# Unrepentant-Atheist/AC-3-ACM-Codec

Measured on AMD Instinct MI355X. Metric: AC-3 5.1@48kHz frames/sec/GPU (decode+encode); achieved HBM GB/s vs peak, higher is better.
Workload: dtype f32+i32

## Files before the change

ac-3-acm-codec_amd/capi.py:

```python
import ctypes
import os
import re

_HERE = os.path.dirname(os.path.abspath(__file__))
LIB_PATH = os.environ.get("AC3MI_LIB") or os.path.join(_HERE, "libac3mi.so")
HEADER_DIR = os.path.join(os.path.dirname(_HERE), "include")

c_void_p, c_int, c_float, c_size_t, c_char_p = (ctypes.c_void_p, ctypes.c_int, ctypes.c_float,
                                                ctypes.c_size_t, ctypes.c_char_p)


class AC3MIError(RuntimeError):
    pass


class XformDescC(ctypes.Structure):
    _fields_ = [("acmod", c_int), ("lfeon", c_int), ("output", c_int), ("bias", c_float)]


class DecodeDescC(ctypes.Structure):
    _fields_ = [("flags", c_int), ("level", c_float), ("bias", c_float), ("dynrng", c_int),
                ("acmod", c_int), ("lfeon", c_int), ("frame_bytes", c_int)]


# ... 179 lines not shown
    lib.ac3mi_syncinfo.argtypes = [c_void_p, ctypes.POINTER(c_int), ctypes.POINTER(c_int), ctypes.POINTER(c_int)]
    lib.ac3mi_decode_planes.argtypes = [ctypes.POINTER(DecodeDescC), ctypes.POINTER(c_int), ctypes.POINTER(c_int)]
    lib.ac3mi_decode_batch.argtypes = [c_void_p, ctypes.POINTER(DecodeDescC), c_void_p, c_int, c_int, c_int,
                                       c_void_p, c_void_p, c_void_p, c_void_p, ctypes.POINTER(DecodeTapsC)]
    lib.ac3mi_decode_s16_batch.argtypes = [c_void_p, ctypes.POINTER(DecodeDescC), c_void_p, c_int, c_int, c_int,
                                           c_void_p, c_void_p, c_void_p, c_void_p]
    lib.ac3mi_encode_frame_bytes.argtypes = [ctypes.POINTER(EncodeDescC)]
    lib.ac3mi_encode_tables.argtypes = [c_void_p] * 5
    lib.ac3mi_encode_batch.argtypes = [c_void_p, ctypes.POINTER(EncodeDescC), c_void_p, c_void_p, c_void_p, c_void_p,
                                       c_void_p, c_int, c_int, c_int, ctypes.POINTER(EncodeTapsC)]
    lib.ac3mi_set_decode_mode.argtypes = [c_void_p, ctypes.c_int]
    if hasattr(lib, "ac3mi_set_fixed_shape"):
        lib.ac3mi_set_fixed_shape.argtypes = [c_void_p, ctypes.c_int]
    if hasattr(lib, "ac3mi_fill_workspaces"):
        lib.ac3mi_fill_workspaces.argtypes = [c_void_p, ctypes.c_int]
    lib.ac3mi_set_decode_crc.argtypes = [c_void_p, ctypes.c_int]
    lib.ac3mi_crc_check_batch.argtypes = [c_void_p, c_void_p, c_int, c_int, c_size_t, c_void_p]
    lib.ac3mi_set_mix_state.argtypes = [c_void_p, c_void_p, c_void_p]
    lib.ac3mi_probe_valu_rate.argtypes = [c_void_p, ctypes.POINTER(ctypes.c_double)]
    lib.ac3mi_probe_salu_rate.argtypes = [c_void_p, ctypes.POINTER(ctypes.c_double)]
    lib.ac3mi_probe_mixed_rate.argtypes = [c_void_p, ctypes.c_int, ctypes.POINTER(ctypes.c_double), ctypes.POINTER(ctypes.c_double)]
    lib.ac3mi_probe_copy_rate.argtypes = [c_void_p, ctypes.c_size_t, ctypes.POINTER(ctypes.c_double)]
    lib.ac3mi_set_tile_frames.argtypes = [c_void_p, ctypes.c_longlong]
    lib.ac3mi_transcode_batch.argtypes = [c_void_p, ctypes.POINTER(DecodeDescC), ctypes.POINTER(EncodeDescC), c_void_p, ctypes.c_int,
                                          ctypes.c_int, ctypes.c_int, c_void_p, c_void_p, c_void_p, c_void_p, c_void_p, c_void_p,
                                          ctypes.c_int, c_void_p]
    _lib = lib
    return lib
```

ac-3-acm-codec_amd/csrc/ac3mi_internal.h:

```cpp
#pragma once
#include <hip/hip_runtime.h>
#include <stdint.h>
#include <array>
#include <string>
#include "../../include/ac3mi.h"
#include "launch_rule.h"

namespace ac3mi {

struct DecTables {
    int8_t la_neg[256];
    uint16_t hth[3][50];
    int8_t width[64];
    uint8_t band_end[30];
    uint8_t band_of_bin[256];
    float qlev[48];
    float qtab[760];
    uint32_t desc[128];
};

struct EncTables {
    int16_t win[256];
    int16_t cos[64], sin[64];
    int16_t xcos[128], xsin[128];
// ... 216 lines not shown
    uint8_t *frames;
    int frame_stride, n_streams, frames_per_stream;
    uint8_t chmap[8];
    int32_t *ws_mdct;
    bool mdct_full_rows = false;
    uint8_t *ws_expo;
    int8_t *ws_shift;
    uint8_t *ws_eexp;
    int16_t *ws_emask;
    uint8_t *ws_strat;
    int32_t *ws_ebits;
    int32_t *ws_snr;
    uint32_t *ws_memo;
    uint8_t *tap_eexp, *tap_bap, *tap_strat;
    int32_t *tap_snr;
    const int32_t *slot;
    int pack_mode = 0;
    const uint32_t *search_hint = nullptr;
    int search_hint_stride = 0;
    uint8_t *ws_bsw = nullptr;
    uint8_t *ws_remat = nullptr;
    int cpl_begf = -1;
    CplWs ws_cpl = {};
    int chbwcod = 50;
    bool bw = false;
    uint32_t bsi = BSI_DEFAULT;
    const uint32_t *bsi_words = nullptr;
    int drc_profile = 0;
    int32_t *drc_state = nullptr;
    int16_t *ws_drc_gain = nullptr;
// ... 62 lines not shown
    ac3mi::DevBuf ws_crc;
    ac3mi::DevBuf ws_bsi;
    ac3mi::DevBuf ws_dyn;
    template <class Ctx> static auto workspaces(Ctx *c)
    {
        return std::array{&c->ws_coef, &c->ws_blksw, &c->ws_draws, &c->ws_split, &c->ws_enc, &c->ws_tc,
                          &c->ws_bsw, &c->ws_remat, &c->ws_cpl, &c->ws_cplr, &c->ws_drc, &c->ws_crc, &c->ws_bsi, &c->ws_dyn};
    }
    const int32_t *slots = nullptr;
    float *mix_pending = nullptr;
    int32_t *mix_flags = nullptr;
    long long tile_frames = 131072;
    int decode_mode = 0;
    int decode_crc = 0;
    int fixed_shape = 1;
    double *loud_tab = nullptr;
    std::string err;
};
```

ac-3-acm-codec_amd/csrc/capi.hip:

```cpp
#include "ac3mi_internal.h"
#include "a52_levels.h"
#include "spec_tables.h"
#include "sync_rule.h"
#include <math.h>
#include <stdio.h>
#include <string.h>
#include <vector>

namespace ac3mi {

static std::string g_err;



static double bessel_i0(double x)
{
    double b = 1;
    for (int i = 100; i > 0; i--) b = b * x / (i * i) + 1;
    return b;
}

void build_host_tables(float *window, float2 *tw_long, float2 *tw_short)
{
    const double pi = 3.14159265358979323846;
// ... 647 lines not shown

int ac3mi_set_decode_mode(ac3mi_ctx *ctx, int mode)
{
    if (!ctx || mode < 0 || mode > 6 || mode == 2) return AC3MI_ERR_ARG;
    ctx->decode_mode = mode;
    return AC3MI_OK;
}

int ac3mi_set_fixed_shape(ac3mi_ctx *ctx, int on)
{
    if (!ctx || on < 0 || on > 1) return AC3MI_ERR_ARG;
    ctx->fixed_shape = on;
    return AC3MI_OK;
}

int ac3mi_set_decode_crc(ac3mi_ctx *ctx, int mode)
{
    if (!ctx || mode < 0 || mode > 2) return AC3MI_ERR_ARG;
    ctx->decode_crc = mode;
    return AC3MI_OK;
}

int ac3mi_set_encode_mode(ac3mi_ctx *ctx, int mode)
{
    if (!ctx || mode < 0 || mode > 2) return AC3MI_ERR_ARG;
    ctx->encode_mode = mode;
    return AC3MI_OK;
}

int ac3mi_set_encode_block_switch(ac3mi_ctx *ctx, int mode)
// ... 346 lines not shown
    E.ws_ebits = ctx->ws_enc.at<int32_t>(W.off_ebits);
    E.ws_snr = ctx->ws_enc.at<int32_t>(W.off_snr);
    E.ws_memo = ctx->ws_enc.at<uint32_t>(W.off_memo);
    if (taps && taps->d_mdct) { E.ws_mdct = taps->d_mdct; E.mdct_full_rows = true; }
    if (taps && taps->d_exponent) E.ws_expo = taps->d_exponent;
    if (taps && taps->d_exp_samples) E.ws_shift = taps->d_exp_samples;
    if (taps && taps->d_encoded_exp) E.ws_eexp = taps->d_encoded_exp;
    E.tap_eexp = taps ? taps->d_encoded_exp : nullptr;
    E.tap_bap = taps ? taps->d_bap : nullptr;
    E.tap_strat = taps ? taps->d_exp_strategy : nullptr;
    E.tap_snr = taps ? taps->d_snroffst : nullptr;
    E.chbwcod = call_chbwcod(ctx, desc, E.cfg.nfbw);
    E.bw = t.bw_mode != 0;
    E.exp_strategy = t.exp_strategy;
    E.pack_mode = ctx->encode_mode;
    E.fixed_shape = ctx->fixed_shape != 0;
    E.slot = ctx->slots;
    return AC3MI_OK;
}

size_t ac3mi_transcode_workspace_plan(size_t frames, int frames_per_stream, int n_in, int nfchans, int n_out)
{
    const bool mantx = dec_mantx(0, frames_per_stream, n_in == n_out, true);
    return (mantx ? 0 : coef_bytes(frames, n_in)) + (zs_off(frames, nfchans) + frames) + split_bytes(frames) +
           s16_ws_bytes(frames, n_out) + enc_ws_layout(frames * 6 * (size_t)n_out).need;
}

int ac3mi_xform_planes(const ac3mi_xform_desc *desc, int *n_in, int *n_out)
{
    MixPlan plan;
    if (!desc) return AC3MI_ERR_ARG;
// ... 640 lines not shown
```

ac-3-acm-codec_amd/csrc/encode.hip:

```cpp
#include "ac3mi_internal.h"
#include "wave_ops.h"
#include "spec_tables.h"
#include "enc_mant.h"
#include "enc_syntax.h"

#include <type_traits>

namespace ac3mi {

#define WAVE_SYNC()                                          \
    do {                                                     \
        __builtin_amdgcn_fence(__ATOMIC_RELEASE, "wavefront"); \
        __builtin_amdgcn_wave_barrier();                     \
        __builtin_amdgcn_fence(__ATOMIC_ACQUIRE, "wavefront"); \
    } while (0)

__device__ __forceinline__ int ilog2u(unsigned v) { return v ? 31 - __builtin_clz(v) : 0; }

__device__ __forceinline__ int wave_sum(int v) { return (int)wave_sum_u32((uint32_t)v); }


struct PackParams {
    const int32_t *mdct;
    const uint8_t *eexp;
    const int16_t *emask;
    const uint8_t *strat;
    const int32_t *ebits;
    const int8_t *shift;
    int32_t *csnr_state;
    const int32_t *slot;
    int32_t *snr;
    uint32_t *memo;
    uint8_t *frames;
    const EncTables *tab;
    uint8_t *tap_eexp;
    uint8_t *tap_bap;
    uint8_t *tap_strat;
    int32_t *tap_snr;
    int n_streams, frames_per_stream, frame_stride;
    int nch, nfbw, lfe, acmod, fscod, halfrate, bsid, frmsizecod, frame_words;
    int nbc;
    int chbwcod;
    uint16_t crc_inv_t[16];
    uint16_t pw1_t[6][16], pw2_t[6][16];
    int c1, c2;
    int frw;
    int marker;
    const uint32_t *hint;
    int hint_stride;
    const uint8_t *bsw;
    const uint8_t *remat;
    CplWs cpl;
    int cpl_begf;
// ... 21 lines not shown
__device__ __forceinline__ uint32_t pack_dynrng(const PackParams &P, size_t fidx, int b, int p)
{
    if constexpr (DW) if (P.dyn) return dyn_sends(P.dyn + fidx * 12, b, p) ? 0x100u | P.dyn[fidx * 12 + 2 * b + p] : 0u;
    if constexpr (MD) if (P.drc && drc_sends(P.drc + fidx * 6, b)) return 0x100u | P.drc[fidx * 6 + b];
    return 0u;
}

struct MaskTabs {
    uint8_t latab[256];
    uint16_t hth[50];
    uint8_t band_of_bin[256];
    uint8_t band_start[52];
};

template <bool CPL>
struct alignas(16) SearchLDS {
    int16_t mask[CPL ? 42 : 36][50];
    uint32_t bitlut[64];
    uint8_t strat[6][6];
    uint8_t band_of_bin[256];
    uint32_t rowdesc[CPL ? 42 : 36];
    uint2 terms[2][50];
};

__device__ __forceinline__ void put_bits(uint32_t *fr, int frw, uint32_t pos, int n, uint32_t v)
{
    if (n <= 0) return;
    const uint32_t w = pos >> 5;
    if (w + 1 >= (uint32_t)frw) return;
    const uint64_t x = (uint64_t)v << (64 - n - (pos & 31));
    const uint32_t hi = (uint32_t)(x >> 32), lo = (uint32_t)x;
    if (hi) atomicOr(&fr[w], hi);
// ... 1315 lines not shown
#define PK_DECL() do { } while (0)
#define PK_T0() do { } while (0)
#define PK_LAP(id) do { } while (0)
#define PK_COUNT(id) do { } while (0)
#define PK_END() do { } while (0)
#endif

#ifndef ENC_NC
#define ENC_NC 3
#endif

#ifndef ENC_SEARCH_LB
#define ENC_SEARCH_LB 4
#endif
template <int PART, bool CPL = false, bool BW = false, bool DRC = false, bool FX = false, bool DW = false>
__global__ __launch_bounds__(64, ENC_SEARCH_LB) void enc_search_kernel(const PackParams P)
{
    static_assert(PART == 1 || PART == 3, "the packers are enc_packf_kernel / enc_packb_kernel");
    static_assert(!DW || DRC, "the array words are costed where the profiles' are");
    static_assert(!FX || (PART == 1 && !CPL && !BW && !DRC), "the fixed 5.1 shape is the plain per-stream search's");
    __shared__ SearchLDS<CPL> L;
    const int lane = threadIdx.x;
    constexpr bool PER_FRAME = PART == 3;
    const int s = PER_FRAME ? (int)(blockIdx.x / (unsigned)P.frames_per_stream) : (int)blockIdx.x;
    const int f_first = PER_FRAME ? (int)(blockIdx.x - (unsigned)s * (unsigned)P.frames_per_stream) : 0;
    const int f_end = PER_FRAME ? f_first + 1 : FX ? 1 : P.frames_per_stream;
    if (s >= P.n_streams) return;

    for (int i = lane; i < 256; i += 64) L.band_of_bin[i] = P.tab->band_of_bin[i];
    {
        const int bp = P.tab->baptab[lane];
        L.bitlut[lane] = (uint32_t)plain_bits(bp) | ((bp == 1) << 9) | ((bp == 2) << 14) | ((bp == 4) << 19);
    }

    const int nch = FX ? 6 : P.nch, nfbw = FX ? 5 : P.nfbw, nbc = FX ? 223 : P.nbc;
    const int acmod = FX ? 7 : P.acmod;
    const bool lfe = FX ? true : P.lfe != 0;
    const int fs = P.frame_words;

    const int sslot = P.slot ? P.slot[s] : s;
    const int cpl_cs = 37 + 12 * P.cpl_begf;
    const int cpl_ce = BW ? 73 + 12 * P.cpl_endf : 217, cpl_nb = BW ? 3 + P.cpl_endf - P.cpl_begf : 15 - P.cpl_begf;
    const int state_in = P.csnr_state[sslot];
    int csnr_prev = state_in & 0xff, fsnr_prev = (state_in >> 8) & 15;
    PK_DECL();

    for (int f = f_first; f < f_end; f++) {
        const size_t fidx = FX ? (size_t)s : (size_t)s * P.frames_per_stream + f;
        PK_T0();
        PK_COUNT(5);
        const uint8_t *ex = P.eexp + fidx * 6 * nch * 256;
        int frame_bits = 0;
        uint64_t run_starts = 0, row_set = 0;
        int ncplrows = 0;
        const bool cplf = CPL && (__builtin_amdgcn_readfirstlane((int)P.cpl.word[fidx]) & 1);
        const uint8_t *cex = cplf ? P.cpl.eexp + fidx * 6 * 256 : ex;
        bool loaded = false;
        auto load_frame = [&]() {
            loaded = true;
            {
                const uint32_t *gm = reinterpret_cast<const uint32_t *>(P.emask + fidx * 6 * nch * 50);
                uint32_t mv[15];
#pragma unroll
                for (int j = 0; j < 15; j++) {
                    const int i = lane + 64 * j;
                    mv[j] = i < 6 * nch * 25 ? gm[i] : 0;
                }
#pragma unroll
                for (int j = 0; j < 15; j++) {
                    const int i = lane + 64 * j;
                    if (i < 6 * nch * 25) reinterpret_cast<uint32_t *>(&L.mask[0][0])[i] = mv[j];
                }
            }
            if (lane < 6 * nch) { const int b = lane / nch, ch = lane - b * nch; L.strat[b][ch] = P.strat[fidx * 6 * nch + lane]; }
            frame_bits = wave_sum(lane < nch ? P.ebits[fidx * nch + lane] : 0);
// ... 30 lines not shown
                    }
                    for (int p = 0; p < np; p++) frame_bits += (compr_word(P, fidx, p) & 0x100u) ? 8 : 0;
                }
                if (!FX && P.remat)
                    for (int b = 1; b < 6; b++) frame_bits += (P.remat[fidx * 6 + b] & 0x10) ? 4 : 0;
                if (CPL && cplf) {
                    frame_bits += syn_priced_cpl(acmod, nfbw, cpl_nb);
                    frame_bits += __builtin_amdgcn_readfirstlane(P.cpl.ebits[fidx]) - 6 * __builtin_popcountll(row_set & fbw_rows);
                    if (P.remat) {
                        const int nrem = syn_cpl_nrem(P.cpl_begf);
                        for (int b = 1; b < 6; b++) frame_bits -= (P.remat[fidx * 6 + b] & 0x10) ? 4 - nrem : 0;
                    }
                }
            }
            if constexpr (CPL) if (cplf) {
                const uint32_t *gm = reinterpret_cast<const uint32_t *>(P.cpl.emask + fidx * 6 * 50);
                for (int i = lane; i < 150; i += 64) reinterpret_cast<uint32_t *>(&L.mask[36][0])[i] = gm[i];
                const int st = lane < 6 ? (int)P.cpl.strat[fidx * 8 + lane] : 0;
                const uint32_t cst = (uint32_t)__ballot(lane < 6 && st != 0) | 0x40u;
                const int n0 = __builtin_popcountll(row_set);
                if (lane < 6 && st != 0) {
                    const int b1 = __builtin_ctz(cst >> (lane + 1)) + lane + 1;
                    const uint32_t cover = ((1u << b1) - 1u) & ~((1u << lane) - 1u);
                    L.rowdesc[n0 + __builtin_popcount(cst & ((1u << lane) - 1u))] = (uint32_t)(lane * 256) | (1u << 15) | (cover << 16) | ((uint32_t)(36 + lane) << 24);
                }
                ncplrows = __builtin_popcount(cst & 0x3fu);
                WAVE_SYNC();
            }
        };
        if (PART != 1 || (!FX && P.tap_strat)) load_frame();

        const uint32_t bandoff = *reinterpret_cast<const uint32_t *>(&L.band_of_bin[4 * lane]);
        SnrSearch ss{csnr_prev, 0, 0, false};
        uint64_t known_c = 0, fits_c = 0;
        uint32_t known_f = 0, fits_f = 0;
        int f_cc = -1;
        if (PART == 1 && !FX && P.memo) {
            const uint32_t *m = P.memo + fidx * 8;
            auto word = [&](int i) { return (uint32_t)__builtin_amdgcn_readfirstlane((int)m[i]); };
            known_c = (uint64_t)word(0) | ((uint64_t)word(1) << 32);
            fits_c = (uint64_t)word(2) | ((uint64_t)word(3) << 32);
            known_f = word(4);
            fits_f = word(5);
            f_cc = (int)word(6);
        }
// ... 3 lines not shown
        int gl = -1, spare_l = 0, gh = -1, spare_h = 0;
        int probe_sweeps = 0;
        auto lookup = [&](int cc, int ff, bool &fits) {
            const int g = 16 * cc + ff;
            if (g <= fit_hi) { fits = true; return true; }
            if (g >= fail_lo) { fits = false; return true; }
            if (((uint32_t)__builtin_amdgcn_readlane((int)costed_map, g >> 5) >> (g & 31)) & 1u) {
                fits = ((uint32_t)__builtin_amdgcn_readlane((int)fits_map, g >> 5) >> (g & 31)) & 1u;
                return true;
            }
            if (ff == 0) { fits = (fits_c >> cc) & 1; return (bool)((known_c >> cc) & 1); }
            fits = (fits_f >> ff) & 1;
            return cc == f_cc && ((known_f >> ff) & 1);
        };
        auto cost_and_record = [&](const int (&cg)[ENC_NC], int n_cand, bool probing) {
            if (!loaded) load_frame();
            int so[ENC_NC];
#pragma unroll
            for (int k = 0; k < ENC_NC; k++) so[k] = ((k < n_cand ? cg[k] : cg[0]) - 240) << 2;
            PK_COUNT(4);
            const int budget = 16 * fs - frame_bits;
            uint32_t acc[6][ENC_NC];
#pragma unroll
            for (int B = 0; B < 6; B++)
#pragma unroll
                for (int c = 0; c < ENC_NC; c++) acc[B][c] = 0;
            {
                const int nrows = __builtin_popcountll(row_set) + (CPL ? ncplrows : 0);
                auto desc_of = [&](int i) { return (uint32_t)__builtin_amdgcn_readfirstlane((int)L.rowdesc[i < nrows ? i : nrows - 1]); };
                auto fetch = [&](uint32_t d) {
// ... 110 lines not shown
                    costed_map |= bit;
                    fits_map |= ok ? bit : 0u;
                }
                {
                    const bool up = ok && g > gl, dn = !ok && (gh < 0 || g < gh);
                    gl = up ? g : gl; spare_l = up ? spare : spare_l;
                    gh = dn ? g : gh; spare_h = dn ? spare : spare_h;
                }
                if (cand_fi == 0) { known_c |= 1ull << cand_ci; fits_c |= (uint64_t)ok << cand_ci; }
                else if (!probing || cand_ci == f_cc) {
                    if (cand_ci != f_cc) { f_cc = cand_ci; known_f = fits_f = 0; }
                    known_f |= 1u << cand_fi;
                    fits_f |= (uint32_t)ok << cand_fi;
                }
            }
        };
        bool first_sweep = true;
        const bool cold_hint = csnr_prev == 40 && fsnr_prev == 0;
        for (;;) {
            int cc, ff;
            bool more;
            while ((more = ss.next(cc, ff))) {
                bool fits;
                if (!lookup(cc, ff, fits)) break;
                if (ss.phase == 0 && !fits) went_down = true;
                if (ss.phase == 1 && fits) went_up = true;
                ss.consume(fits);
            }
            if (!more) break;
            int cg[ENC_NC], n_cand = 0;
#pragma unroll
            for (int k = 0; k < ENC_NC; k++) cg[k] = -1;
            auto add = [&](int g) {
// ... 749 lines not shown
    PackParams P;
    P.mdct = E.ws_mdct;
    P.eexp = E.ws_eexp;
    P.emask = E.ws_emask;
    P.strat = E.ws_strat;
    P.ebits = E.ws_ebits;
    P.shift = E.ws_shift;
    P.csnr_state = E.csnr;
    P.slot = E.slot;
    P.frames = E.frames;
    P.tab = tab.enc;
    P.tap_eexp = E.tap_eexp;
    P.tap_bap = E.tap_bap;
    P.tap_strat = E.tap_strat;
    P.tap_snr = E.tap_snr;
    P.n_streams = E.n_streams;
    P.frames_per_stream = E.frames_per_stream;
    P.frame_stride = E.frame_stride;
    P.nch = c.nch;
    P.nfbw = c.nfbw;
    P.lfe = c.lfe;
    P.acmod = c.acmod;
    P.fscod = c.fscod;
    P.halfrate = c.halfrate;
    P.bsid = c.bsid;
    P.frmsizecod = c.frmsizecod;
    P.frame_words = c.frame_words;
    P.nbc = R.nbc;
    P.chbwcod = E.chbwcod;
    const int fs = c.frame_words, fs58 = (fs >> 1) + (fs >> 3);
// ... 93 lines not shown
```

ac-3-acm-codec_amd/csrc/wave_ops.h:

```cpp
#pragma once
#include <hip/hip_runtime.h>
#include <stdint.h>

namespace ac3mi {

__device__ __forceinline__ uint32_t wave_incl_scan_u32(uint32_t v)
{
    v += (uint32_t)__builtin_amdgcn_update_dpp(0, (int)v, 0x111, 0xf, 0xf, true);
    v += (uint32_t)__builtin_amdgcn_update_dpp(0, (int)v, 0x112, 0xf, 0xf, true);
    v += (uint32_t)__builtin_amdgcn_update_dpp(0, (int)v, 0x114, 0xf, 0xf, true);
    v += (uint32_t)__builtin_amdgcn_update_dpp(0, (int)v, 0x118, 0xf, 0xf, true);
    v += (uint32_t)__builtin_amdgcn_update_dpp(0, (int)v, 0x142, 0xa, 0xf, false);
    v += (uint32_t)__builtin_amdgcn_update_dpp(0, (int)v, 0x143, 0xc, 0xf, false);
    return v;
}

__device__ __forceinline__ uint32_t wave_last(uint32_t v) { return (uint32_t)__builtin_amdgcn_readlane((int)v, 63); }

__device__ __forceinline__ uint32_t wave_sum_u32(uint32_t v) { return wave_last(wave_incl_scan_u32(v)); }

__device__ __forceinline__ uint32_t wave_or_u32(uint32_t v)
{
    v |= (uint32_t)__builtin_amdgcn_update_dpp(0, (int)v, 0x111, 0xf, 0xf, true);
    v |= (uint32_t)__builtin_amdgcn_update_dpp(0, (int)v, 0x112, 0xf, 0xf, true);
    v |= (uint32_t)__builtin_amdgcn_update_dpp(0, (int)v, 0x114, 0xf, 0xf, true);
    v |= (uint32_t)__builtin_amdgcn_update_dpp(0, (int)v, 0x118, 0xf, 0xf, true);
    v |= (uint32_t)__builtin_amdgcn_update_dpp(0, (int)v, 0x142, 0xa, 0xf, false);
    v |= (uint32_t)__builtin_amdgcn_update_dpp(0, (int)v, 0x143, 0xc, 0xf, false);
// ... 65 lines not shown
```

ac-3-acm-codec_amd/engine.py:

```python
import ctypes
from dataclasses import dataclass

from . import capi


@dataclass
class XformDesc:
    acmod: int = 7
    lfeon: int = 1
    output: int = 7 | 16
    bias: float = 0.0

    def c(self):
        return capi.XformDescC(self.acmod, self.lfeon, self.output, self.bias)


@dataclass
class DecodeDesc:
    flags: int = 7 | 16
    level: float = 1.0
    bias: float = 0.0
    dynrng: int = 1
    acmod: int = 7
    lfeon: int = 1
# ... 300 lines not shown
        self.lib.ac3mi_workspace_bytes.restype = ctypes.c_size_t
        return int(self.lib.ac3mi_workspace_bytes(ctypes.c_void_p(self.ctx)))

    def fill_workspaces(self, byte):
        self._check(self.lib.ac3mi_fill_workspaces(ctypes.c_void_p(self.ctx), int(byte)))

    def set_tile_frames(self, frames):
        self._check(self.lib.ac3mi_set_tile_frames(ctypes.c_void_p(self.ctx), int(frames)))

    def set_decode_mode(self, mode):
        self._check(self.lib.ac3mi_set_decode_mode(ctypes.c_void_p(self.ctx), int(mode)))

    def set_fixed_shape(self, on):
        self._check(self.lib.ac3mi_set_fixed_shape(ctypes.c_void_p(self.ctx), int(on)))

    def set_decode_crc(self, mode):
        self._check(self.lib.ac3mi_set_decode_crc(ctypes.c_void_p(self.ctx), int(mode)))

    def crc_check_batch(self, frames, frame_bytes=None, out=None, wait_torch=True):
        import torch
        assert frames.dtype == torch.uint8 and frames.is_contiguous() and frames.is_cuda and frames.dim() >= 2
        stride = frames.shape[-1]
        n = frames.numel() // stride if stride else 0
        if out is None:
            out = torch.zeros(tuple(frames.shape[:-1]), dtype=torch.uint8, device=frames.device)
        assert out.dtype == torch.uint8 and out.is_contiguous() and out.numel() == n
        self._drain_torch(wait_torch)
        self._check(self.lib.ac3mi_crc_check_batch(ctypes.c_void_p(self.ctx), ctypes.c_void_p(frames.data_ptr()), int(stride),
                                                   int(stride if frame_bytes is None else frame_bytes), ctypes.c_size_t(n),
                                                   ctypes.c_void_p(out.data_ptr())))
# ... 279 lines not shown
```

include/ac3mi.h:

```cpp
#ifndef AC3MI_H
#define AC3MI_H

#include <stddef.h>
#include <stdint.h>

#ifdef __cplusplus
extern "C" {
#endif

#define AC3MI_CHANNEL 0
#define AC3MI_MONO 1
#define AC3MI_STEREO 2
#define AC3MI_3F 3
#define AC3MI_2F1R 4
#define AC3MI_3F1R 5
#define AC3MI_2F2R 6
#define AC3MI_3F2R 7
#define AC3MI_CHANNEL1 8
#define AC3MI_CHANNEL2 9
#define AC3MI_DOLBY 10
#define AC3MI_CHANNEL_MASK 15
#define AC3MI_LFE 16
#define AC3MI_ADJUST_LEVEL 32

// ... 33 lines not shown
    int output;
    float bias;
} ac3mi_xform_desc;

int ac3mi_set_state_slots(ac3mi_ctx *ctx, const int32_t *d_slots);

int ac3mi_set_mix_state(ac3mi_ctx *ctx, float *d_pending, int32_t *d_flags);

#define AC3MI_STATUS_REUSE0 0x200u
int ac3mi_set_decode_mode(ac3mi_ctx *ctx, int mode);

int ac3mi_set_fixed_shape(ac3mi_ctx *ctx, int on);

int ac3mi_fill_workspaces(ac3mi_ctx *ctx, int byte);

#define AC3MI_STATUS_CRC1 0x400u
#define AC3MI_STATUS_CRC2 0x800u
int ac3mi_set_decode_crc(ac3mi_ctx *ctx, int mode);

int ac3mi_crc_check_batch(ac3mi_ctx *ctx, const uint8_t *d_frames, int frame_stride, int frame_bytes, size_t n_frames,
                          uint8_t *d_verdict);

#define AC3MI_BSI_NOT_READ 0x80u
#define AC3MI_BSI_OVERRUN 0x40u
#define AC3MI_BSI_COMPRE 0x001u
#define AC3MI_BSI_LANGCODE 0x002u
#define AC3MI_BSI_AUDPRODIE 0x004u
#define AC3MI_BSI_COMPR2E 0x008u
#define AC3MI_BSI_LANGCOD2E 0x010u
#define AC3MI_BSI_AUDPRODI2E 0x020u
// ... 207 lines not shown
```

Measured before the change: 9.294 million.

## Cost sixteen SNR offsets per sweep with histogram window search in encoder

Replaces the per-candidate bit costing in the per-stream encoder SNR search (PART 1) with a windowed sweep. Each pass costs 16 consecutive SNR offsets at once using wave scans and LDS histograms of the bit-count steps, and a predictive rule (linear interpolation, hints) picks the next window. The mask rows are no longer staged in LDS; masks are read straight from global memory. Launch bounds for the fixed 5.1 shape go up to 7 waves per EU, and a debug curve tap plus a Python simulator are added. This aims to cut the number of search iterations per frame, at the cost of more per-sweep work and register pressure.

```diff
diff --git a/ac-3-acm-codec_amd/capi.py b/ac-3-acm-codec_amd/capi.py
--- a/ac-3-acm-codec_amd/capi.py
+++ b/ac-3-acm-codec_amd/capi.py
@@ -217,6 +217,8 @@
         lib.ac3mi_set_fixed_shape.argtypes = [c_void_p, ctypes.c_int]
     if hasattr(lib, "ac3mi_fill_workspaces"):
         lib.ac3mi_fill_workspaces.argtypes = [c_void_p, ctypes.c_int]
+    if hasattr(lib, "ac3mi_debug_search_curve"):
+        lib.ac3mi_debug_search_curve.argtypes = [c_void_p, c_void_p]
     lib.ac3mi_set_decode_crc.argtypes = [c_void_p, ctypes.c_int]
     lib.ac3mi_crc_check_batch.argtypes = [c_void_p, c_void_p, c_int, c_int, c_size_t, c_void_p]
     lib.ac3mi_set_mix_state.argtypes = [c_void_p, c_void_p, c_void_p]
diff --git a/ac-3-acm-codec_amd/csrc/ac3mi_internal.h b/ac-3-acm-codec_amd/csrc/ac3mi_internal.h
--- a/ac-3-acm-codec_amd/csrc/ac3mi_internal.h
+++ b/ac-3-acm-codec_amd/csrc/ac3mi_internal.h
@@ -254,6 +254,7 @@
     uint32_t *ws_memo;
     uint8_t *tap_eexp, *tap_bap, *tap_strat;
     int32_t *tap_snr;
+    int32_t *tap_curve = nullptr;
     const int32_t *slot;
     int pack_mode = 0;
     const uint32_t *search_hint = nullptr;
@@ -346,6 +347,7 @@
     int decode_mode = 0;
     int decode_crc = 0;
     int fixed_shape = 1;
+    int32_t *debug_search_curve = nullptr;
     double *loud_tab = nullptr;
     std::string err;
 };
diff --git a/ac-3-acm-codec_amd/csrc/capi.hip b/ac-3-acm-codec_amd/csrc/capi.hip
--- a/ac-3-acm-codec_amd/csrc/capi.hip
+++ b/ac-3-acm-codec_amd/csrc/capi.hip
@@ -685,6 +685,13 @@
     return AC3MI_OK;
 }
 
+int ac3mi_debug_search_curve(ac3mi_ctx *ctx, int32_t *d_curve)
+{
+    if (!ctx) return AC3MI_ERR_ARG;
+    ctx->debug_search_curve = d_curve;
+    return AC3MI_OK;
+}
+
 int ac3mi_set_decode_crc(ac3mi_ctx *ctx, int mode)
 {
     if (!ctx || mode < 0 || mode > 2) return AC3MI_ERR_ARG;
@@ -1061,7 +1068,8 @@
     E.bw = t.bw_mode != 0;
     E.exp_strategy = t.exp_strategy;
     E.pack_mode = ctx->encode_mode;
-    E.fixed_shape = ctx->fixed_shape != 0;
+    E.tap_curve = ctx->debug_search_curve;
+    E.fixed_shape = ctx->fixed_shape != 0 && !ctx->debug_search_curve;
     E.slot = ctx->slots;
     return AC3MI_OK;
 }
diff --git a/ac-3-acm-codec_amd/csrc/encode.hip b/ac-3-acm-codec_amd/csrc/encode.hip
--- a/ac-3-acm-codec_amd/csrc/encode.hip
+++ b/ac-3-acm-codec_amd/csrc/encode.hip
@@ -3,6 +3,7 @@
 #include "spec_tables.h"
 #include "enc_mant.h"
 #include "enc_syntax.h"
+#include "snr_window.h"
 
 #include <type_traits>
 
@@ -37,6 +38,7 @@
     uint8_t *tap_bap;
     uint8_t *tap_strat;
     int32_t *tap_snr;
+    int32_t *tap_curve;
     int n_streams, frames_per_stream, frame_stride;
     int nch, nfbw, lfe, acmod, fscod, halfrate, bsid, frmsizecod, frame_words;
     int nbc;
@@ -88,8 +90,15 @@
 };
 
 template <bool CPL>
-struct alignas(16) SearchLDS {
+struct SearchMaskRows {
     int16_t mask[CPL ? 42 : 36][50];
+};
+struct SearchWindowBufs {
+    alignas(16) uint32_t scan[4 + 256];
+    alignas(16) uint32_t hist[4][6][15][2];
+};
+template <bool CPL, bool WIN>
+struct alignas(16) SearchLDS : std::conditional_t<WIN, SearchWindowBufs, SearchMaskRows<CPL>> {
     uint32_t bitlut[64];
     uint8_t strat[6][6];
     uint8_t band_of_bin[256];
@@ -1435,12 +1444,13 @@
 #define ENC_SEARCH_LB 4
 #endif
 template <int PART, bool CPL = false, bool BW = false, bool DRC = false, bool FX = false, bool DW = false>
-__global__ __launch_bounds__(64, ENC_SEARCH_LB) void enc_search_kernel(const PackParams P)
+__global__ __launch_bounds__(64, FX ? 7 : ENC_SEARCH_LB) void enc_search_kernel(const PackParams P)
 {
     static_assert(PART == 1 || PART == 3, "the packers are enc_packf_kernel / enc_packb_kernel");
     static_assert(!DW || DRC, "the array words are costed where the profiles' are");
     static_assert(!FX || (PART == 1 && !CPL && !BW && !DRC), "the fixed 5.1 shape is the plain per-stream search's");
-    __shared__ SearchLDS<CPL> L;
+    constexpr bool WIN = PART == 1;
+    __shared__ SearchLDS<CPL, WIN> L;
     const int lane = threadIdx.x;
     constexpr bool PER_FRAME = PART == 3;
     const int s = PER_FRAME ? (int)(blockIdx.x / (unsigned)P.frames_per_stream) : (int)blockIdx.x;
@@ -1452,6 +1462,13 @@
     {
         const int bp = P.tab->baptab[lane];
         L.bitlut[lane] = (uint32_t)plain_bits(bp) | ((bp == 1) << 9) | ((bp == 2) << 14) | ((bp == 4) << 19);
+    }
+    int band_lo = 0, band_hi = 0;
+    if constexpr (WIN) {
+        const int b = lane < 50 ? lane : 49;
+        band_lo = 3 + P.tab->band_start[b];
+        band_hi = 3 + (b < 49 ? P.tab->band_start[b + 1] : 256);
+        if (lane == 0) L.scan[3] = 0;
     }
 
     const int nch = FX ? 6 : P.nch, nfbw = FX ? 5 : P.nfbw, nbc = FX ? 223 : P.nbc;
@@ -1479,7 +1496,7 @@
         bool loaded = false;
         auto load_frame = [&]() {
             loaded = true;
-            {
+            if constexpr (!WIN) {
                 const uint32_t *gm = reinterpret_cast<const uint32_t *>(P.emask + fidx * 6 * nch * 50);
                 uint32_t mv[15];
 #pragma unroll
@@ -1540,8 +1557,10 @@
                 }
             }
             if constexpr (CPL) if (cplf) {
-                const uint32_t *gm = reinterpret_cast<const uint32_t *>(P.cpl.emask + fidx * 6 * 50);
-                for (int i = lane; i < 150; i += 64) reinterpret_cast<uint32_t *>(&L.mask[36][0])[i] = gm[i];
+                if constexpr (!WIN) {
+                    const uint32_t *gm = reinterpret_cast<const uint32_t *>(P.cpl.emask + fidx * 6 * 50);
+                    for (int i = lane; i < 150; i += 64) reinterpret_cast<uint32_t *>(&L.mask[36][0])[i] = gm[i];
+                }
                 const int st = lane < 6 ? (int)P.cpl.strat[fidx * 8 + lane] : 0;
                 const uint32_t cst = (uint32_t)__ballot(lane < 6 && st != 0) | 0x40u;
                 const int n0 = __builtin_popcountll(row_set);
@@ -1554,7 +1573,7 @@
                 WAVE_SYNC();
             }
         };
-        if (PART != 1 || (!FX && P.tap_strat)) load_frame();
+        if (PART != 1 || FX || P.tap_strat) load_frame();
 
         const uint32_t bandoff = *reinterpret_cast<const uint32_t *>(&L.band_of_bin[4 * lane]);
         SnrSearch ss{csnr_prev, 0, 0, false};
@@ -1588,6 +1607,7 @@
             return cc == f_cc && ((known_f >> ff) & 1);
         };
         auto cost_and_record = [&](const int (&cg)[ENC_NC], int n_cand, bool probing) {
+          if constexpr (!WIN) {
             if (!loaded) load_frame();
             int so[ENC_NC];
 #pragma unroll
@@ -1728,9 +1748,188 @@
                     fits_f |= (uint32_t)ok << cand_fi;
                 }
             }
+          }
+        };
+        int win_sweeps = 0, win_slope15 = 0, win_cmin = 1 << 20, win_cmax = -1;
+        auto cost_window = [&](int lo) {
+          if constexpr (WIN) {
+            if (!loaded) load_frame();
+            PK_COUNT(4);
+            const int so_lo = win_snroffset(lo);
+            const int budget = 16 * fs - frame_bits;
+            uint32_t acc[6];
+#pragma unroll
+            for (int B = 0; B < 6; B++) acc[B] = 0;
+            static_assert(sizeof L.hist == 180 * sizeof(uint4), "cleared as 180 uint4");
+#pragma unroll
+            for (int i = 0; i < 3; i++)
+                if (lane + 64 * i < 180) reinterpret_cast<uint4 *>(&L.hist[0][0][0][0])[lane + 64 * i] = make_uint4(0, 0, 0, 0);
+            {
+                const int nrows = __builtin_popcountll(row_set) + (CPL ? ncplrows : 0);
+                auto desc_of = [&](int i) { return (uint32_t)__builtin_amdgcn_readfirstlane((int)L.rowdesc[i < nrows ? i : nrows - 1]); };
+                auto fetch = [&](uint32_t d) {
+                    if constexpr (CPL) return *reinterpret_cast<const uint32_t *>(((d & (1u << 15)) ? cex : ex) + (d & 0x3fffu) + 4 * lane);
+                    else return *reinterpret_cast<const uint32_t *>(ex + (d & 0x3fffu) + 4 * lane);
+                };
+                const int bl = lane < 50 ? lane : 49;
+                const int16_t *gmask = P.emask + fidx * 6 * nch * 50 + bl;
+                auto mask_of = [&](uint32_t d) {
+                    if constexpr (CPL) if (d & (1u << 15)) return (int)P.cpl.emask[(fidx * 6 + ((d >> 24) - 36)) * 50 + bl];
+                    return (int)gmask[(d >> 24) * 50u];
+                };
+                uint32_t d0 = desc_of(0), d1 = desc_of(1), d2 = desc_of(2);
+                uint32_t ev = fetch(d0), ev1 = fetch(d1), ev2 = fetch(d2);
+                int t1c = 0, t2c = 0;
+                auto terms = [&](int m, int buf, int &t1, int &t2) {
+                    int k0;
+                    win_steps(m - so_lo, k0, t1, t2);
+                    const int D = win_term(k0);
+                    if (lane < 50) L.terms[buf][lane] = make_uint2((uint32_t)(D & 0xffff) | ((uint32_t)(D + 4) << 16), (uint32_t)((D + 8) & 0xffff));
+                };
+                int mv1 = mask_of(d1);
+                terms(mask_of(d0), 0, t1c, t2c);
+                auto beyond = [&](int n) { const int k = n - 4 * lane; return k >= 4 ? 0u : k <= 0 ? 0xffffffffu : 0xffffffffu << (8 * k); };
+                const uint32_t um_fbw = beyond(nbc), um_lfe = beyond(7);
+                uint32_t boff[4];
+#pragma unroll
+                for (int j = 0; j < 4; j++) boff[j] = ((bandoff >> (8 * j)) & 0xffu) * 8u;
+#pragma unroll 1
+                for (int i = 0; i < nrows; i++) {
+                    const uint32_t d3 = desc_of(i + 3);
+                    const uint32_t ev3 = fetch(d3);
+                    const int mv2 = mask_of(d2);
+                    const char *Tr = reinterpret_cast<const char *>(&L.terms[i & 1][0]);
+                    uint32_t em;
+                    if constexpr (CPL) {
+                        const uint32_t um_cch = beyond(cpl_cs), um_cpl = ~beyond(cpl_cs) | beyond(cpl_ce);
+                        em = ev | ((d0 & (1u << 14)) ? um_lfe : (d0 & (1u << 15)) ? um_cpl : (d0 & (1u << 22)) ? um_cch : um_fbw);
+                    } else {
+                        em = ev | ((d0 & (1u << 14)) ? um_lfe : um_fbw);
+                    }
+                    uint32_t p[3][4];
+#pragma unroll
+                    for (int j = 0; j < 4; j++) {
+                        const uint32_t e16 = __umul24((em >> (8 * j)) & 0xffu, 0x00100010u);
+                        const uint2 t = *reinterpret_cast<const uint2 *>(Tr + boff[j]);
+                        pk2 a01 = __builtin_bit_cast(pk2, t.x) - __builtin_bit_cast(pk2, e16);
+                        pk2 a2 = __builtin_bit_cast(pk2, t.y) - __builtin_bit_cast(pk2, e16);
+                        a01 = __builtin_elementwise_min(__builtin_elementwise_max(a01, (pk2){0, 0}), (pk2){252, 252});
+                        a2 = __builtin_elementwise_min(__builtin_elementwise_max(a2, (pk2){0, 0}), (pk2){252, 252});
+                        const char *lut = reinterpret_cast<const char *>(&L.bitlut[0]);
+                        const uint32_t v0 = *reinterpret_cast<const uint32_t *>(lut + (uint16_t)a01.x);
+                        const uint32_t v1 = *reinterpret_cast<const uint32_t *>(lut + (uint16_t)a01.y);
+                        const uint32_t v2 = *reinterpret_cast<const uint32_t *>(lut + (uint16_t)a2.x);
+                        p[0][j] = j ? p[0][j - 1] + v0 : v0;
+                        p[1][j] = j ? p[1][j - 1] + v1 : v1;
+                        p[2][j] = j ? p[2][j - 1] + v2 : v2;
+                    }
+#pragma unroll
+                    for (int B = 0; B < 6; B++) {
+                        const uint32_t in_run = (d0 >> (16 + B)) & 1u;
+                        asm("v_mad_u32_u24 %0, %1, %2, %0" : "+v"(acc[B]) : "v"(p[0][3]), "s"(in_run));
+                    }
+                    uint32_t W[3];
+#pragma unroll
+                    for (int c = 0; c < 3; c++) {
+                        const uint32_t incl = wave_incl_scan_u32(p[c][3]);
+                        const uint32_t before = incl - p[c][3];
+                        *reinterpret_cast<uint4 *>(&L.scan[4 + 4 * lane]) = make_uint4(before + p[c][0], before + p[c][1], before + p[c][2], incl);
+                        W[c] = L.scan[band_hi] - L.scan[band_lo];
+                    }
+                    {
+                        const uint32_t cover = (d0 >> 16) & 0x3fu;
+                        const int b_in = __builtin_ctz(cover), b_out = b_in + __builtin_popcount(cover);
+                        const uint32_t a0 = win_wide_a(W[0]), a1 = win_wide_a(W[1]), a2 = win_wide_a(W[2]);
+                        const uint32_t b0 = win_wide_b(W[0]), b1 = win_wide_b(W[1]), b2 = win_wide_b(W[2]);
+                        const bool s1 = lane < 50 && t1c < WIN_N && ((a1 ^ a0) | (b1 ^ b0)) != 0, s2 = lane < 50 && t2c < WIN_N && ((a2 ^ a1) | (b2 ^ b1)) != 0;
+                        uint32_t *h1 = &L.hist[lane & 3][b_in][s1 ? t1c - 1 : 0][0], *h2 = &L.hist[lane & 3][b_in][s2 ? t2c - 1 : 0][0];
+                        if (s1) { atomicAdd(h1, a1 - a0); atomicAdd(h1 + 1, b1 - b0); }
+                        if (s2) { atomicAdd(h2, a2 - a1); atomicAdd(h2 + 1, b2 - b1); }
+                        if (b_out < 6) {
+                            const int behind = (b_out - b_in) * 30;
+                            if (s1) { atomicAdd(h1 + behind, a0 - a1); atomicAdd(h1 + behind + 1, b0 - b1); }
+                            if (s2) { atomicAdd(h2 + behind, a1 - a2); atomicAdd(h2 + behind + 1, b1 - b2); }
+                        }
+                    }
+                    if (i + 1 < nrows) terms(mv1, (i + 1) & 1, t1c, t2c);
+                    d0 = d1; d1 = d2; d2 = d3;
+                    ev = ev1; ev1 = ev2; ev2 = ev3;
+                    mv1 = mv2;
+                }
+            }
+            int spare, extra6;
+            {
+                const int t = lane & 15;
+                uint32_t run_a = 0, run_b = 0, total = 0, x6 = 0;
+#pragma unroll
+                for (int B = 0; B < 6; B++) {
+                    const uint32_t base_a = wave_sum_u32(win_wide_a(acc[B])), base_b = wave_sum_u32(win_wide_b(acc[B]));
+#pragma unroll
+                    for (int c = 0; c < 4; c++) {
+                        const uint2 h = *reinterpret_cast<const uint2 *>(&L.hist[c][B][t ? t - 1 : 0][0]);
+                        run_a += t ? h.x : 0u;
+                        run_b += t ? h.y : 0u;
+                    }
+                    uint32_t e6;
+                    total += win_block_bits(base_a + row_incl_scan_u32(run_a), base_b + row_incl_scan_u32(run_b), e6);
+                    x6 += e6;
+                }
+                spare = budget - (int)total;
+                extra6 = (int)x6;
+            }
+            {
+                const uint32_t fits16 = (uint32_t)__ballot(spare >= 0) & 0xffffu, fails16 = fits16 ^ 0xffffu;
+                const uint32_t sure_fit = (uint32_t)__ballot(6 * spare >= 414 - extra6) & 0xffffu;
+                const uint32_t sure_fail = (uint32_t)__ballot(6 * spare < -extra6) & 0xffffu;
+                const int g_fit = sure_fit ? lo + 31 - __builtin_clz(sure_fit) : -1, g_fail = sure_fail ? lo + __builtin_ctz(sure_fail) : 1 << 20;
+                fit_hi = g_fit > fit_hi ? g_fit : fit_hi;
+                fail_lo = g_fail < fail_lo ? g_fail : fail_lo;
+                {
+                    const uint64_t c16 = (uint64_t)0xffffu << (lo & 31), f16 = (uint64_t)fits16 << (lo & 31);
+                    const int w = lo >> 5;
+                    costed_map |= lane == w ? (uint32_t)c16 : lane == w + 1 ? (uint32_t)(c16 >> 32) : 0u;
+                    fits_map |= lane == w ? (uint32_t)f16 : lane == w + 1 ? (uint32_t)(f16 >> 32) : 0u;
+                }
+                {
+                    const int il = fits16 ? 31 - __builtin_clz(fits16) : 0, ih = fails16 ? __builtin_ctz(fails16) : 0;
+                    const int sp_l = __builtin_amdgcn_readlane(spare, il), sp_h = __builtin_amdgcn_readlane(spare, ih);
+                    const bool up = fits16 && lo + il > gl, dn = fails16 && (gh < 0 || lo + ih < gh);
+                    gl = up ? lo + il : gl; spare_l = up ? sp_l : spare_l;
+                    gh = dn ? lo + ih : gh; spare_h = dn ? sp_h : spare_h;
+                }
+                win_slope15 = __builtin_amdgcn_readlane(spare, 0) - __builtin_amdgcn_readlane(spare, 15);
+                win_cmin = lo < win_cmin ? lo : win_cmin;
+                win_cmax = lo + 15 > win_cmax ? lo + 15 : win_cmax;
+                if constexpr (!FX) if (P.tap_curve && lane < WIN_N) {
+                    P.tap_curve[(fidx * 1024 + lo + lane) * 2] = spare;
+                    P.tap_curve[(fidx * 1024 + lo + lane) * 2 + 1] = extra6;
+                }
+            }
+          }
         };
         bool first_sweep = true;
         const bool cold_hint = csnr_prev == 40 && fsnr_prev == 0;
+        if constexpr (WIN) {
+            for (;;) {
+                int cc, ff;
+                bool more;
+                while ((more = ss.next(cc, ff))) {
+                    bool fits;
+                    if (!lookup(cc, ff, fits)) break;
+                    ss.consume(fits);
+                }
+                if (!more) break;
+                int lo;
+                if (win_sweeps == 0) {
+                    const int hint0 = (cold_hint && P.hint) ? (int)__builtin_amdgcn_readfirstlane((int)P.hint[fidx * (size_t)P.hint_stride]) : 0;
+                    lo = win_first_lo(hint0, cold_hint, 16 * csnr_prev + fsnr_prev);
+                } else {
+                    lo = win_next_lo(win_sweeps, gl, spare_l, gh, spare_h, win_slope15, win_cmin, win_cmax, 16 * cc + ff);
+                }
+                win_sweeps++;
+                cost_window(lo);
+            }
+        } else
         for (;;) {
             int cc, ff;
             bool more;
@@ -2510,6 +2709,7 @@
     P.tap_bap = E.tap_bap;
     P.tap_strat = E.tap_strat;
     P.tap_snr = E.tap_snr;
+    P.tap_curve = E.tap_curve;
     P.n_streams = E.n_streams;
     P.frames_per_stream = E.frames_per_stream;
     P.frame_stride = E.frame_stride;
diff --git a/ac-3-acm-codec_amd/csrc/snr_window.h b/ac-3-acm-codec_amd/csrc/snr_window.h
--- /dev/null
+++ b/ac-3-acm-codec_amd/csrc/snr_window.h
@@ -0,0 +1,92 @@
+#pragma once
+#include <stdint.h>
+
+#ifndef __HIPCC__
+#ifndef __host__
+#define __host__
+#endif
+#ifndef __device__
+#define __device__
+#endif
+#endif
+
+namespace ac3mi {
+
+constexpr int WIN_N = 16;
+constexpr int WIN_NEVER = 16;
+constexpr int WIN_LO_MAX = 1008;
+
+__host__ __device__ inline int win_snroffset(int g) { return (g - 240) * 4; }
+
+__host__ __device__ inline void win_steps(int x, int &k0, int &t1, int &t2)
+{
+    const int k = x >> 5;
+    k0 = k < 0 ? 0 : k;
+    const int s = ((x & 31) >> 2) + 1;
+    t1 = k >= 1 ? s : WIN_NEVER;
+    t2 = k >= 2 ? s + 8 : WIN_NEVER;
+}
+__host__ __device__ inline int win_taken(int t, int t1, int t2) { return (t >= t1) + (t >= t2); }
+
+__host__ __device__ inline int win_term(int k0) { return 320 - 4 * k0; }
+__host__ __device__ inline int win_addr(int k0, int j, int e)
+{
+    const int a = 80 - k0 + j - 4 * e;
+    return a < 0 ? 0 : a > 63 ? 63 : a;
+}
+
+__host__ __device__ inline uint32_t win_wide_a(uint32_t w) { return (w & 0x1ffu) | ((w & 0x3e00u) << 6); }
+__host__ __device__ inline uint32_t win_wide_b(uint32_t w) { return ((w >> 14) & 0x1fu) | ((w >> 8) & 0xf800u); }
+
+__host__ __device__ inline uint32_t win_block_bits(uint32_t a, uint32_t b, uint32_t &extra6)
+{
+    const uint32_t n1 = a >> 15, n2 = b & 0x7ffu, n4 = b >> 11;
+    const uint32_t t = 5u * (((n1 + 2u) * 0xaaabu) >> 17) + 7u * (((n2 + 2u) * 0xaaabu) >> 17) + 7u * ((n4 + 1u) >> 1);
+    extra6 = 6u * t - (10u * n1 + 14u * n2 + 21u * n4);
+    return (a & 0x7fffu) + t;
+}
+
+__host__ __device__ inline int win_clamp_lo(int lo) { return lo < 0 ? 0 : lo > WIN_LO_MAX ? WIN_LO_MAX : lo; }
+
+constexpr int WIN_HINT_BELOW = 5;
+constexpr int WIN_COLD_LO = 176;
+constexpr int WIN_WARM_BELOW = 6;
+constexpr int WIN_LINE_SWEEPS = 4;
+constexpr int WIN_ASK_SWEEPS = 7;
+
+__host__ __device__ inline int win_first_lo(int hint, bool cold, int g_prev)
+{
+    return win_clamp_lo(hint > 0 ? hint - WIN_HINT_BELOW : cold ? WIN_COLD_LO : g_prev - WIN_WARM_BELOW);
+}
+
+__host__ __device__ inline int win_next_lo(int sweeps, int gl, int sl, int gh, int sh, int slope15, int cmin, int cmax, int gq)
+{
+    if (sweeps >= WIN_ASK_SWEEPS) return win_clamp_lo(gq - 8);
+    const int around = win_clamp_lo(gq < cmin ? cmin - WIN_N : gq > cmax ? cmax + 1 : gq - 8);
+    if (gl >= 0 && gh >= 0) {
+        if (gh <= gl + 1 || gq <= gl || gq >= gh) return around;
+        const int w = gh - gl;
+        if (w - 1 <= WIN_N) return win_clamp_lo(gl + 1);
+        int est = gl + (w >> 1);
+        if (sweeps < WIN_LINE_SWEEPS) est = gl + (w * sl + ((sl - sh) >> 1)) / (sl - sh);
+        int lo = est - 8;
+        lo = lo < gl + 1 ? gl + 1 : lo;
+        lo = lo > gh - WIN_N ? gh - WIN_N : lo;
+        return win_clamp_lo(lo);
+    }
+    if (gh < 0 ? gq <= gl : gq >= gh) return around;
+    if (gh < 0) {
+        int est = slope15 > 0 ? gl + (15 * sl) / slope15 : 1023;
+        if (sweeps >= WIN_LINE_SWEEPS) est = gl + ((1024 - gl) >> 1);
+        est = est > 1023 ? 1023 : est;
+        const int lo = est - 8;
+        return win_clamp_lo(lo < gl + 1 ? gl + 1 : lo);
+    }
+    int est = slope15 > 0 ? gh - (15 * -sh) / slope15 : 0;
+    if (sweeps >= WIN_LINE_SWEEPS) est = gh >> 1;
+    est = est < 0 ? 0 : est;
+    const int lo = est - 7;
+    return win_clamp_lo(lo > gh - WIN_N ? gh - WIN_N : lo);
+}
+
+}
diff --git a/ac-3-acm-codec_amd/csrc/wave_ops.h b/ac-3-acm-codec_amd/csrc/wave_ops.h
--- a/ac-3-acm-codec_amd/csrc/wave_ops.h
+++ b/ac-3-acm-codec_amd/csrc/wave_ops.h
@@ -12,6 +12,15 @@
     v += (uint32_t)__builtin_amdgcn_update_dpp(0, (int)v, 0x118, 0xf, 0xf, true);
     v += (uint32_t)__builtin_amdgcn_update_dpp(0, (int)v, 0x142, 0xa, 0xf, false);
     v += (uint32_t)__builtin_amdgcn_update_dpp(0, (int)v, 0x143, 0xc, 0xf, false);
+    return v;
+}
+
+__device__ __forceinline__ uint32_t row_incl_scan_u32(uint32_t v)
+{
+    v += (uint32_t)__builtin_amdgcn_update_dpp(0, (int)v, 0x111, 0xf, 0xf, true);
+    v += (uint32_t)__builtin_amdgcn_update_dpp(0, (int)v, 0x112, 0xf, 0xf, true);
+    v += (uint32_t)__builtin_amdgcn_update_dpp(0, (int)v, 0x114, 0xf, 0xf, true);
+    v += (uint32_t)__builtin_amdgcn_update_dpp(0, (int)v, 0x118, 0xf, 0xf, true);
     return v;
 }
 
diff --git a/ac-3-acm-codec_amd/engine.py b/ac-3-acm-codec_amd/engine.py
--- a/ac-3-acm-codec_amd/engine.py
+++ b/ac-3-acm-codec_amd/engine.py
@@ -338,6 +338,9 @@
     def set_fixed_shape(self, on):
         self._check(self.lib.ac3mi_set_fixed_shape(ctypes.c_void_p(self.ctx), int(on)))
 
+    def debug_search_curve(self, curve):
+        self._check(self.lib.ac3mi_debug_search_curve(ctypes.c_void_p(self.ctx), ctypes.c_void_p(curve.data_ptr() if curve is not None else None)))
+
     def set_decode_crc(self, mode):
         self._check(self.lib.ac3mi_set_decode_crc(ctypes.c_void_p(self.ctx), int(mode)))
 
diff --git a/include/ac3mi.h b/include/ac3mi.h
--- a/include/ac3mi.h
+++ b/include/ac3mi.h
@@ -71,6 +71,8 @@
 
 int ac3mi_fill_workspaces(ac3mi_ctx *ctx, int byte);
 
+int ac3mi_debug_search_curve(ac3mi_ctx *ctx, int32_t *d_curve);
+
 #define AC3MI_STATUS_CRC1 0x400u
 #define AC3MI_STATUS_CRC2 0x800u
 int ac3mi_set_decode_crc(ac3mi_ctx *ctx, int mode);
diff --git a/profiles/search_window_sim.py b/profiles/search_window_sim.py
--- /dev/null
+++ b/profiles/search_window_sim.py
@@ -0,0 +1,123 @@
+#!/usr/bin/env python3
+import os
+import sys
+
+sys.path.insert(0, os.path.dirname(os.path.abspath(__file__)))
+from search_sim import Search, curves, reference, run as run3
+
+WIN_N = 16
+HINT_BELOW, COLD_LO, WARM_BELOW = 5, 176, 6
+LINE_SWEEPS, ASK_SWEEPS = 4, 7
+
+
+def clamp_lo(lo):
+    return 0 if lo < 0 else 1008 if lo > 1008 else lo
+
+
+def first_lo(hint, cold, g_prev, hint_below=HINT_BELOW, cold_lo=COLD_LO, warm_below=WARM_BELOW):
+    return clamp_lo(hint - hint_below if hint and hint > 0 else cold_lo if cold else g_prev - warm_below)
+
+
+def next_lo(sweeps, gl, sl, gh, sh, slope15, cmin, cmax, gq):
+    if sweeps >= ASK_SWEEPS: return clamp_lo(gq - 8)
+    around = clamp_lo(cmin - WIN_N if gq < cmin else cmax + 1 if gq > cmax else gq - 8)
+    if gl >= 0 and gh >= 0:
+        if gh <= gl + 1 or gq <= gl or gq >= gh: return around
+        w = gh - gl
+        if w - 1 <= WIN_N: return clamp_lo(gl + 1)
+        est = gl + (w >> 1)
+        if sweeps < LINE_SWEEPS: est = gl + (w * sl + ((sl - sh) >> 1)) // (sl - sh)
+        lo = min(max(est - 8, gl + 1), gh - WIN_N)
+        return clamp_lo(lo)
+    if (gq <= gl) if gh < 0 else (gq >= gh): return around
+    if gh < 0:
+        est = gl + (15 * sl) // slope15 if slope15 > 0 else 1023
+        if sweeps >= LINE_SWEEPS: est = gl + ((1024 - gl) >> 1)
+        est = min(est, 1023)
+        return clamp_lo(max(est - 8, gl + 1))
+    est = gh - (15 * -sh) // slope15 if slope15 > 0 else 0
+    if sweeps >= LINE_SWEEPS: est = gh >> 1
+    est = max(est, 0)
+    return clamp_lo(min(est - 7, gh - WIN_N))
+
+
+def run(curve, start, hint=None, fsnr_prev=0, **first_kw):
+    extra = curve.extra
+    costed = {}
+    fit_hi, fail_lo = -1, 1 << 20
+    gl = gh = -1
+    sl = sh = 0
+    slope15 = 0
+    cmin, cmax = 1 << 20, -1
+    ss = Search(start)
+    sweeps = 0
+    cold = start == 40 and fsnr_prev == 0
+
+    def lookup(g):
+        if g <= fit_hi: return True
+        if g >= fail_lo: return False
+        return costed.get(g)
+
+    while True:
+        q = None
+        while True:
+            q = ss.next()
+            if q is None: break
+            v = lookup(16 * q[0] + q[1])
+            if v is None: break
+            ss.consume(v)
+        if q is None: break
+        gq = 16 * q[0] + q[1]
+        if sweeps == 0:
+            lo = first_lo(hint if cold else None, cold, 16 * start + fsnr_prev, **first_kw)
+        else:
+            lo = next_lo(sweeps, gl, sl, gh, sh, slope15, cmin, cmax, gq)
+        sweeps += 1
+        assert sweeps <= 64, "the window rule does not end"
+        for g in range(lo, lo + WIN_N):
+            sp, e6 = int(curve[g]), int(extra[g])
+            costed[g] = sp >= 0
+            if 6 * sp >= 414 - e6 and g > fit_hi: fit_hi = g
+            if 6 * sp < -e6 and g < fail_lo: fail_lo = g
+            if sp >= 0 and g > gl: gl, sl = g, sp
+            if sp < 0 and (gh < 0 or g < gh): gh, sh = g, sp
+        slope15 = int(curve[lo]) - int(curve[lo + 15])
+        cmin, cmax = min(cmin, lo), max(cmax, lo + 15)
+    return sweeps, (ss.c, ss.f)
+
+
+def table(name, sweeps, base):
+    n = len(sweeps)
+    hist = {}
+    for s in sweeps: hist[s] = hist.get(s, 0) + 1
+    print("%-34s window %.2f sweeps per frame (three-offset policy %.2f); histogram %s" % (
+        name, sum(sweeps) / n, sum(base) / n, " ".join("%d:%d" % (k, hist[k]) for k in sorted(hist))))
+
+
+if __name__ == "__main__":
+    n = int(sys.argv[1]) if len(sys.argv) > 1 else 60
+    tr, trb, cold, coldb, warm, warmb, land, delta = [], [], [], [], [], [], [], []
+    for seed in (7, 99):
+        for c, g_src in curves(n, seed=seed, second_gen=True, with_source=True):
+            want = reference(c, 40)
+            sw, got = run(c, 40, hint=g_src)
+            assert got == want
+            tr.append(sw); trb.append(run3(c, 40, "probe", hint=g_src)[0])
+            delta.append(16 * want[0] + want[1] - g_src)
+        prev = None
+        for c in curves(n, seed=seed):
+            want = reference(c, 40)
+            sw, got = run(c, 40)
+            assert got == want
+            cold.append(sw); coldb.append(run3(c, 40, "probe")[0])
+            land.append(16 * want[0] + want[1])
+            if prev is not None:
+                sw, got = run(c, prev[0], fsnr_prev=prev[1])
+                assert got == reference(c, prev[0])
+                warm.append(sw); warmb.append(run3(c, prev[0], "probe")[0])
+            prev = want
+    table("transcoded (hint = source offsets)", tr, trb)
+    table("fresh, cold", cold, coldb)
+    table("fresh, warm", warm, warmb)
+    print("the re-encode lands %d .. %d steps from its source; fresh frames land at g = %d .. %d, mean %.0f" % (
+        min(delta), max(delta), min(land), max(land), sum(land) / len(land)))
```

Measured after the change: 9.607 million, median of 6. 3.4% higher.
